# dscripka/openWakeWord

Measured on NVIDIA H100. Metric: 80ms audio-frames/sec (concurrent streams), higher is better.
Workload: dtype f16 operands / f32 accumulate (mel, BN, LayerNorm, sigmoid in f32; heads' first layer as fp16 hi/lo split = f32-grade)

## Files before the change

openwakeword_b200/csrc/cnn_tc.cu:

```cuda
#include "oww_internal.h"
#include "tc_common.cuh"
#include <algorithm>
#include <cmath>
#include <cstring>

namespace {

struct Tc0Args {
    WindowSrc src;
    int n_windows; int T_out;
    const float* w; const float* scale; const float* bias;
    __half* out; int64_t plane;
};

__global__ void __launch_bounds__(256) tc_conv0_kernel(Tc0Args a) {
    __shared__ float s_w[9 * 24];
    __shared__ float s_s[24], s_b[24];
    for (int i = threadIdx.x; i < 9 * 24; i += 256) s_w[i] = a.w[i];
    if (threadIdx.x < 24) { s_s[threadIdx.x] = a.scale[threadIdx.x]; s_b[threadIdx.x] = a.bias[threadIdx.x]; }
    __syncthreads();
    constexpr int Wp = 33;
    const int T = a.T_out;
    const int64_t total = (int64_t)a.n_windows * T * Wp;
    for (int64_t p = (int64_t)blockIdx.x * 256 + threadIdx.x; p < total; p += (int64_t)gridDim.x * 256) {
// ... 230 lines not shown
                        reinterpret_cast<uint32_t*>(o + (int64_t)(a.cg_out + g) * a.out_plane)[q] = lw;
                        if (po == 0) reinterpret_cast<uint32_t*>(o + (int64_t)(a.cg_out + g) * a.out_plane - 1)[q] = 0u;
                    }
                }
            }
        }
    }
}

struct TcBlkArgs {
    const __half* in; LateLay lay;
    const __half* w; const float* scale; const float* bias;
    int n, W, rows_new;
    int m_valid, tap;
    int pool_f;
    int cg_in, cg_out, apply_act, n_tiles;
    float* out_f32;
    __half* out[3]; int out_toff[3];
    LateLay out_lay;
    int64_t out_plane;
};

template <int CGP, int NP>
__global__ void __launch_bounds__(kTcThreads, 1) tc_conv_blk_kernel(TcBlkArgs a) {
    extern __shared__ __align__(128) uint8_t smem[];
    constexpr int W_TERM = 3 * CGP * NP * 16;
    constexpr int W_BYTES = 2 * W_TERM;
    uint8_t* w_smem = smem;
    const int units = a.lay.units;
    const int half_bytes = CGP * units * 16;
    uint8_t* a_smem = smem + W_BYTES;
    uint64_t* bars = reinterpret_cast<uint64_t*>(a_smem + 2 * half_bytes);
    float* s_sb = reinterpret_cast<float*>(bars + 6);
    for (int i = threadIdx.x; i < NP; i += kTcThreads) { s_sb[i] = a.scale[i]; s_sb[NP + i] = a.bias[i]; }

    const int warp = threadIdx.x >> 5, lane = threadIdx.x & 31;
    const uint32_t bar0 = smem_u32(bars);
    auto full_bar = [&](int h) { return bar0 + 8u * h; };
    auto empty_bar = [&](int h) { return bar0 + 8u * (2 + h); };
    const uint32_t wfull_bar = bar0 + 8u * 4;

    if (threadIdx.x == 0) {
        for (int h = 0; h < 2; ++h) { mbar_init(full_bar(h), 1); mbar_init(empty_bar(h), 8); }
        mbar_init(wfull_bar, 1);
        asm volatile("fence.mbarrier_init.release.cluster;" ::: "memory");
    }
    if (a.cg_in < CGP)
        for (int h = 0; h < 2; ++h) {
// ... 54 lines not shown
                        for (int wt = 0; wt < (h == 0 ? 2 : 1); ++wt) {
                            const uint32_t w_t = w_addr + (wt == 1 ? (uint32_t)W_TERM : 0u);
                            const uint64_t ad = make_desc(a_addr + (uint32_t)h * (uint32_t)half_bytes + (uint32_t)(2 * qq) * lbo_a + (uint32_t)j * tap16,
                                                          lbo_a, 128u);
                            const uint64_t bd = make_desc(w_t + (uint32_t)((j * CGP + 2 * qq) * NP) * 16u, NP * 16u, 128u);
                            wg_mma<NP>(acc, ad, bd, (h | j | qq | wt) != 0);
                        }
                    }
                }
                wg_commit();
                wg_wait_all();
                __syncwarp();
                if (lane == 0) mbar_arrive(empty_bar(h));
            }
            phase ^= 1;

#pragma unroll
            for (int i = 0; i < 2; ++i) {
                const int t = tr[i], sl = slr[i], f = fr[i];
                const int n = tile * a.lay.S + sl;
                const bool live = okr[i] && n < a.n;
                if (a.out_f32) {
                    if (!live || f != 0) continue;
                    float* o = a.out_f32 + ((int64_t)n * a.rows_new + t) * 96;
#pragma unroll
                    for (int j = 0; j < NP / 8; ++j) {
                        const int c = j * 8 + 2 * q;
                        if (c >= 96) continue;
                        float2 r;
                        r.x = fmaf(acc[4 * j + 2 * i], s_sb[c], s_sb[NP + c]);
// ... 123 lines not shown
                        8 * (2 * stages + 2) + 2 * NP * sizeof(float);
    if (smem > 227 * 1024) return oww_fail(ctx, OWW_EUNSUPPORTED, "tensor-core conv tile does not fit shared memory (%zu bytes)", smem);
    const uint32_t bit = 1u << (((CGP / 2 + NP / 16) + (TERMS == 3 ? 16 : 0)) & 31);
    if (!(ctx->tc_attr_mask & bit)) {
        OWW_CUDA(ctx, cudaFuncSetAttribute(tc_conv_kernel<CGP, NP, TERMS>, cudaFuncAttributeMaxDynamicSharedMemorySize, 227 * 1024));
        ctx->tc_attr_mask |= bit;
    }
    int grid = ctx->sm_count < a.n_tiles ? ctx->sm_count : a.n_tiles;
    tc_conv_kernel<CGP, NP, TERMS><<<grid, kTcThreads, smem, s>>>(a);
    OWW_LAUNCH_CHECK(ctx);
    return OWW_OK;
}

template <int CGP, int NP>
int launch_tc_blk(oww_ctx* ctx, const TcBlkArgs& a, cudaStream_t s) {
    const size_t smem = (size_t)2 * 3 * CGP * NP * 16 + (size_t)2 * CGP * a.lay.units * 16 + 8 * 6 + 2 * NP * sizeof(float);
    if (smem > 227 * 1024) return oww_fail(ctx, OWW_EUNSUPPORTED, "blocked late conv tile does not fit shared memory (%zu bytes)", smem);
    const uint32_t bit = 1u << (CGP / 2 + NP / 16);
    if (!(ctx->tc_blk_attr_mask & bit)) {
        OWW_CUDA(ctx, cudaFuncSetAttribute(tc_conv_blk_kernel<CGP, NP>, cudaFuncAttributeMaxDynamicSharedMemorySize, 227 * 1024));
        ctx->tc_blk_attr_mask |= bit;
    }
    const int grid = ctx->sm_count < a.n_tiles ? ctx->sm_count : a.n_tiles;
    OWW_CUDA(ctx, oww_launch_pdl(ctx->late_pdl, tc_conv_blk_kernel<CGP, NP>, dim3(grid), dim3(kTcThreads), smem, s, a));
    OWW_LAUNCH_CHECK(ctx);
    return OWW_OK;
}

}

int oww_tc_pack_weights(oww_ctx* ctx, const float* h_blob) {
// ... 161 lines not shown
            if (rc) return rc;
            if (cap->late && (rc = oww_late_capture(ctx, li + 1, bufs[cur ^ 1], in_plane, T, W, s))) return rc;
        }
        if (li == stop_layer && !last) {
            const int64_t total = (int64_t)n * T * W * L.cout;
            tc_unpack_kernel<<<(unsigned)((total + 255) / 256), 256, 0, s>>>(bufs[cur ^ 1], in_plane, d_dbg, n, T, W, L.cout, out_split ? 1 : 0);
            OWW_LAUNCH_CHECK(ctx);
            return OWW_OK;
        }
    }
    return OWW_OK;
}

namespace {

__global__ void late_capture_kernel(const uint4* planes, int64_t plane_pitch, int T, int Wp, int n_planes, uint4* tmpl) {
    const int total = n_planes * 2 * Wp;
    for (int i = blockIdx.x * blockDim.x + threadIdx.x; i < total; i += gridDim.x * blockDim.x) {
        const int f = i % Wp, r = (i / Wp) % 2, pl = i / (2 * Wp);
        tmpl[i] = planes[(int64_t)pl * plane_pitch + kGuard + (int64_t)(T - 2 + r) * Wp + f];
    }
}

}

int oww_late_alloc(oww_ctx* ctx) {
    for (auto& X : ctx->late_x) for (auto& b : X.buf) { cudaFree(b); b = nullptr; }
    cudaFree(ctx->d_late_tmp); ctx->d_late_tmp = nullptr;
    cudaFree(ctx->d_late_template); ctx->d_late_template = nullptr;
    ctx->late_active = false;
// ... 14 lines not shown
        LateLay& Y = X.lay;
        Y.kh3 = kh3 ? 1 : 0; Y.T = rows + (kh3 ? 2 : 0); Y.Wq = kh3 ? W : W + 1;
        Y.S = std::max(1, 128 / (rows * Y.Wq));
        if (kh3) while (Y.S > 1 && Y.T * Y.S * W > 256) Y.S /= 2;
        const int tap = kh3 ? Y.S * W : 1;
        Y.units = round8(std::max((kh3 ? 0 : 1) + Y.T * Y.S * Y.Wq, 2 * tap + 128));
        Y.blk_stride = (int64_t)2 * X.cg * Y.units;
        const size_t buf_units = (size_t)((n + Y.S - 1) / Y.S) * Y.blk_stride;
        X.tmpl_off = kh3 ? (int)tmpl_units : -1;
        if (kh3) tmpl_units += (size_t)2 * X.cg * 2 * (W + 1);
        for (int k = 0; k < X.n_buf; ++k) {
            OWW_CUDA(ctx, cudaMalloc(&X.buf[k], buf_units * 16));
            OWW_CUDA(ctx, cudaMemset(X.buf[k], 0, buf_units * 16));
        }
        if (C.pool_t) {
            const size_t u = (size_t)2 * (C.cout / 8) * ((kGuard + (size_t)n * rows * (W + 1) + kGuardBack + 7) & ~(size_t)7);
            if (u > tmp_units) tmp_units = u;
            rows /= C.pool_t; W /= C.pool_f;
        }
    }
    if (tmp_units) {
        OWW_CUDA(ctx, cudaMalloc(&ctx->d_late_tmp, tmp_units * 16));
        OWW_CUDA(ctx, cudaMemset(ctx->d_late_tmp, 0, tmp_units * 16));
    }
    OWW_CUDA(ctx, cudaMalloc(&ctx->d_late_template, std::max<size_t>(tmpl_units, 1) * 16));
    OWW_CUDA(ctx, cudaMemset(ctx->d_late_template, 0, std::max<size_t>(tmpl_units, 1) * 16));
    ctx->late_step = 0;
    ctx->late_active = true;
    return OWW_OK;
}

int oww_late_chain(oww_ctx* ctx, float* d_emb, cudaStream_t s) {
// ... 12 lines not shown
                toff[m] = 2 - m * Y.rows_new;
            }
        };
        const int64_t tmp_plane = (int64_t)((kGuard + (int64_t)n * T_out * (W + 1) + kGuardBack + 7) & ~7LL);
        TcBlkArgs b;
        std::memset(&b, 0, sizeof(b));
        b.in = reinterpret_cast<const __half*>(X.buf[X.n_buf == 1 ? 0 : (int)(k % X.n_buf)]);
        b.lay = X.lay;
        b.w = reinterpret_cast<const __half*>(ctx->d_tc_w3) + 2 * ctx->tc_w_off[l];
        b.scale = ctx->d_tc_sb3 + ctx->tc_sb_off[l]; b.bias = b.scale + np;
        b.n = n; b.W = W; b.rows_new = T_out;
        b.m_valid = T_out * X.lay.S * X.lay.Wq;
        b.tap = C.kh == 3 ? X.lay.S * W : 1;
        b.cg_in = cg; b.cg_out = C.cout / 8; b.apply_act = last ? 0 : 1;
        b.n_tiles = (n + X.lay.S - 1) / X.lay.S;
        const bool fuse_pool = !last && C.pool_t == 1 && C.pool_f == 2 && X.lay.kh3 && (W & 1) == 0;
        if (last) {
            b.out_f32 = d_emb;
        } else if (C.pool_t && !fuse_pool) {
            b.out[0] = reinterpret_cast<__half*>(ctx->d_late_tmp);
            b.out_plane = tmp_plane;
        } else {
            const oww_ctx::LateTensor& Y = ctx->late_x[l + 1];
            route(Y, b.out, b.out_toff);
            b.out_lay = Y.lay;
            b.pool_f = fuse_pool ? 2 : 0;
        }
        int rc;
        if (cgp == 4 && np == 48) rc = launch_tc_blk<4, 48>(ctx, b, s);
        else if (cgp == 6 && np == 48) rc = launch_tc_blk<6, 48>(ctx, b, s);
        else if (cgp == 6 && np == 80) rc = launch_tc_blk<6, 80>(ctx, b, s);
        else if (cgp == 10 && np == 80) rc = launch_tc_blk<10, 80>(ctx, b, s);
        else if (cgp == 10 && np == 96) rc = launch_tc_blk<10, 96>(ctx, b, s);
        else if (cgp == 12 && np == 96) rc = launch_tc_blk<12, 96>(ctx, b, s);
        else rc = oww_fail(ctx, OWW_EUNSUPPORTED, "no block-major late conv instance for cgp=%d np=%d", cgp, np);
        if (rc) return rc;
        if (C.pool_t && !last && !fuse_pool) {
            const oww_ctx::LateTensor& Y = ctx->late_x[l + 1];
            PoolOut po{{nullptr, nullptr, nullptr}, {0, 0, 0}, Y.lay};
            route(Y, po.p, po.toff);
            const int cgo = C.cout / 8;
// ... 24 lines not shown
```

openwakeword_b200/csrc/cnn_tc_inc.cu:

```cuda
#include "oww_internal.h"
#include "tc_common.cuh"
#include "mel_device.cuh"
#include <cmath>
#include <cstring>
#include <type_traits>

namespace {

constexpr int kIncEpiWarps = 16;
constexpr int kIncThreads = kIncEpiWarps * 32;
constexpr int kIncMaxG = 7;
constexpr int kMelNF = 2;

__device__ __forceinline__ __half2 u32_as_half2(uint32_t v) {
    return __halves2half2(__ushort_as_half((unsigned short)(v & 0xFFFFu)), __ushort_as_half((unsigned short)(v >> 16)));
}

struct IncArgs {
    IncPlan plan;
    const float* mel; const int* mel_count; int64_t mel_stride; int mel_mask; int back;
    const float* w0; const float* s0; const float* b0;
    const uint8_t* wblob;
    const uint4* tails_in; uint4* tails_out;
    float* emb;
// ... 10 lines not shown
    int hring_off, hslot_bytes, hns;
    const Gate* gates; int n_gates;
    uint4* gx; LateLay gx_lay;
};

__device__ __forceinline__ int head_rows(int slot_bytes, int K, int D) {
    const int r = (slot_bytes / (D * 4)) & ~3;
    return r < K ? r : K;
}

template <int kNL>
__global__ void __launch_bounds__(kIncThreads, 1) tc_inc_kernel(const __grid_constant__ IncArgs a) {
    extern __shared__ __align__(128) uint8_t smem[];
    const IncPlan& P = a.plan;
    const int NL = kNL ? kNL : P.n_layers;
    const int G = P.G;
    uint64_t* bars = reinterpret_cast<uint64_t*>(smem);
    float* s_l0 = reinterpret_cast<float*>(smem + 704);
    uint4* act0 = reinterpret_cast<uint4*>(smem + 2048);

    const int warp = __shfl_sync(0xffffffffu, (int)(threadIdx.x >> 5), 0);
    const int lane = threadIdx.x & 31;
    const uint32_t bar0 = smem_u32(bars);
    auto wfull = [&](int i) { return bar0 + 8u * i; };
    const uint32_t tails_bar = bar0 + 8u * 2;
    auto hfull = [&](int i) { return bar0 + 8u * (3 + i); };
    auto hempty = [&](int i) { return bar0 + 8u * (7 + i); };

    if (threadIdx.x == 0) {
        for (int i = 0; i < 2; ++i) mbar_init(wfull(i), 1);
        mbar_init(tails_bar, 1);
        for (int i = 0; i < 4; ++i) { mbar_init(hfull(i), 1); mbar_init(hempty(i), kIncEpiWarps); }
        asm volatile("fence.mbarrier_init.release.cluster;" ::: "memory");
    }
    for (int i = threadIdx.x; i < 9 * 24; i += kIncThreads) s_l0[i] = a.w0[i];
    if (threadIdx.x < 24) { s_l0[216 + threadIdx.x] = a.s0[threadIdx.x]; s_l0[240 + threadIdx.x] = a.b0[threadIdx.x]; }
    asm volatile("fence.proxy.async.shared::cta;" ::: "memory");
    __syncthreads();

    auto load_weights = [&](int l) {
        mbar_expect_tx(wfull(l & 1), (uint32_t)P.L[l].w_bytes);
        bulk_g2s(smem_u32(smem + P.L[l].w_smem), a.wblob + P.L[l].w_off, (uint32_t)P.L[l].w_bytes, wfull(l & 1));
    };
    if (threadIdx.x == 0 && (int)blockIdx.x < P.n_groups) { load_weights(1); load_weights(2); }

    int hq_head = 0, hq_layer = 0, hq_row = 0, hchunk_p = 0;
    auto issue_head_chunk = [&]() -> bool {
        if (hq_head >= a.n_heads) return false;
        const HeadDev& H = a.heads[hq_head];
        const int slot = hchunk_p % a.hns;
        mbar_wait(hempty(slot), ((hchunk_p / a.hns) & 1) ^ 1);
        uint32_t bytes; const float* src;
        if (hq_layer == 0) {
            bytes = (uint32_t)(96 * H.dims[1]) * 4u;
            src = H.blob + H.w_off[0] + (int64_t)hq_row * 96 * H.dims[1];
            if (++hq_row == H.n_in) { hq_row = 0; hq_layer = 1; }
        } else {
            const int K = H.dims[hq_layer], D = H.dims[hq_layer + 1];
            const int rows = head_rows(a.hslot_bytes, K, D);
// ... 13 lines not shown
    uint32_t epi_tails_par = 0, mma_tails_par = 0;
    uint32_t hf_par = 0; int hchunk_e = 0;
    for (int grp = blockIdx.x; grp < P.n_groups; grp += gridDim.x) {
        const uint4* tin = a.tails_in + (int64_t)grp * P.tail_units;
        uint4* tout = a.tails_out + (int64_t)grp * P.tail_units;
        int* s_cnt = reinterpret_cast<int*>(smem + 512);
        int* s_live = s_cnt + 16;
        float* s_mel = reinterpret_cast<float*>(smem + P.scratch_off + 6144);
        if (a.dbg_clock && blockIdx.x == 0 && grp == 0 && et == 0) a.dbg_clock[101] = clock64();
        named_bar_sync(2, kIncEpiWarps * 32);
        if (et < G) {
            const int b = grp * G + et;
            s_live[et] = b < a.B && (!a.live_chunks || a.live_chunks[b] >= a.live_min);
        }
        named_bar_sync(2, kIncEpiWarps * 32);
        if (a.fused) {
            uint8_t* sc = smem + P.scratch_off;
            float2* s_tw = reinterpret_cast<float2*>(sc);
            float* s_win = reinterpret_cast<float*>(sc + 4096);
            uint8_t* s_work = smem + 2048 + warp * (kMelNF * kMelFrameScratch);
            float* s_floor = s_mel + G * 256;
            int seen_v = 1;
            for (int i = et; i < 512; i += kIncEpiWarps * 32) { s_tw[i] = a.mel_twiddle[i]; s_win[i] = a.mel_window[i]; }
            if (et < G) {
                const int b = grp * G + et;
                s_cnt[et] = s_live[et] ? a.mel_count_rw[b] : 0;
                s_cnt[8 + et] = s_live[et] ? a.feat_count[b] : 0;
                seen_v = s_live[et] ? a.seen[b] : 1;
                s_live[8 + et] = s_live[et] && seen_v == 0;
            }
            named_bar_sync(2, kIncEpiWarps * 32);
// ... 90 lines not shown
            if (l == 0) {
                const int Wp = 33, NP2 = 17;
                for (int q = et; q < 8 * G * NP2; q += kIncEpiWarps * 32) {
                    const int j = q % NP2, tg = q / NP2, g = tg % G, t = tg / G;
                    const int f0 = 2 * j;
                    const int b = grp * G + g;
                    uint4* o = nx + 1 + tg * Wp + f0;
                    const uint4 z = make_uint4(0, 0, 0, 0);
                    if (j == 16) { o[0] = z; o[L.nx_pitch] = z; o[2 * L.nx_pitch] = z; continue; }
                    if (!s_live[g]) {
                        o[0] = z; o[L.nx_pitch] = z; o[2 * L.nx_pitch] = z;
                        o[1] = z; o[L.nx_pitch + 1] = z; o[2 * L.nx_pitch + 1] = z;
                        continue;
                    }
                    const float* base = a.mel + (int64_t)b * a.mel_stride;
                    const int row0 = (a.fused ? s_cnt[g] - 2 : a.mel_count[b] - a.back - 10) + t;
                    float x[3][4];
#pragma unroll
                    for (int dt = 0; dt < 3; ++dt) {
                        const float* rp = (a.fused && t + dt >= 2) ? s_mel + (g * 8 + t + dt - 2) * 32
                                                                   : base + (int64_t)((row0 + dt) & a.mel_mask) * 32;
#pragma unroll
                        for (int i = 0; i < 4; ++i) {
                            const int ff = f0 + i - 1;
                            x[dt][i] = (ff >= 0 && ff < 32) ? rp[ff] : 0.f;
                        }
                    }
#pragma unroll
                    for (int pl = 0; pl < 3; ++pl) {
                        __half2 h0[4], h1[4];
#pragma unroll
                        for (int u = 0; u < 4; ++u) {
                            float v0[2], v1[2];
#pragma unroll
                            for (int e = 0; e < 2; ++e) {
// ... 84 lines not shown
                };
                auto epi_item = [&](auto nc_const, auto final_const, const float* acc, int it) {
                    constexpr int NP = decltype(nc_const)::value;
                    constexpr bool kFinal = decltype(final_const)::value;
                    const int t64 = it / n_chunks, c0 = (it - t64 * n_chunks) * NP;
#pragma unroll
                    for (int i = 0; i < 2; ++i) {
                        const int m = t64 * 64 + wq * 16 + (lane >> 2) + 8 * i;
                        if (m >= lM) continue;
                        const int tg = (int)__umulhi((uint32_t)m, wp_magic);
                        const int f = m - tg * lWp;
                        const int g = G > 1 ? tg - (int)__umulhi((uint32_t)tg, g_magic) * G : 0;
                        const bool live = s_live[g] != 0;
                        if constexpr (kFinal) {
                            if (f != 0 || !live) continue;
                            float* o = a.fused ? a.feat_ring + (int64_t)(grp * G + g) * a.feat_stride + (int64_t)(s_cnt[8 + g] & a.feat_mask) * 96
                                               : a.emb + (int64_t)(grp * G + g) * 96;
#pragma unroll
                            for (int j = 0; j < NP / 8; ++j) {
                                const int c = c0 + j * 8 + 2 * q;
                                float2 r;
                                r.x = fmaf(acc[4 * j + 2 * i], sb[c], sb[lnp + c]);
                                r.y = fmaf(acc[4 * j + 2 * i + 1], sb[c + 1], sb[lnp + c + 1]);
                                *reinterpret_cast<float2*>(o + c) = r;
                            }
                            continue;
                        }
                        const bool pad = f == lW;
                        uint4* d0 = dst + (1 + t_off_units + m);
                        const bool keep_tail = !lpool && ltail >= 0 && m >= tail_start && live;
                        uint4* t0 = tout + (ltail + (m - tail_start));
// ... 118 lines not shown
                    }
                }
            }
            if (L.nx_tail_off >= 0) epi_tails_par ^= 1;
            asm volatile("fence.proxy.async.shared::cta;" ::: "memory");
            named_bar_sync(1, kIncEpiWarps * 32);
            if (l > 0 && et == 0) {
                if (l + 2 < NL) load_weights(l + 2);
                else if (grp + (int)gridDim.x < P.n_groups) {
                    if (l == NL - 2 && (l & 1)) load_weights(1);
                    if (l == NL - 1) { if (l & 1) load_weights(1); load_weights(2); }
                }
            }
        }
        if (a.dbg_clock && blockIdx.x == 0 && grp == 0 && et == 0) a.dbg_clock[OWW_N_CONV] = clock64();
        if (a.fused && NL == OWW_N_CONV) {
            named_bar_sync(2, kIncEpiWarps * 32);
            if (a.n_heads > 0) {
            if (et == 0) {
                hq_head = hq_layer = hq_row = 0;
                for (int i = 0; i < a.hns && issue_head_chunk(); ++i) {}
            }
            auto refill_head_ring = [&]() {
                while (hchunk_p < hchunk_e - 1 + max(a.hns, 2) && issue_head_chunk()) {}
            };
            const int NI = a.max_n_in;
            float* feats = reinterpret_cast<float*>(smem + 2048);
            float* red = feats + G * NI * 96;
            float* hA = red + 4 * G * 128;
            float* hB = hA + G * 256;
            for (int i0 = et; i0 < G * NI * 24; i0 += 4 * kIncEpiWarps * 32) {
// ... 279 lines not shown
        if (L.nx_base + size_nx[l] > hi) hi = L.nx_base + size_nx[l];
        act_high[l] = kActBase + hi * 16;
    }
    auto wsz = [&](int l) { return l >= 1 && l < NL ? (P.L[l].w_bytes + 127) & ~127 : 0; };
    for (int l = 1; l < NL; ++l) {
        const int above = wsz(l + 1) > wsz(l - 1) ? wsz(l + 1) : wsz(l - 1);
        P.L[l].w_smem = (l & 1) ? kTop - wsz(l) : kTop - above - wsz(l);
    }
    for (int l = 1; l < NL; ++l) {
        int w_low = P.L[l].w_smem;
        if (l + 1 < NL && P.L[l + 1].w_smem < w_low) w_low = P.L[l + 1].w_smem;
        if (act_high[l] > w_low || act_high[l - 1] > P.L[l].w_smem)
            return oww_fail(ctx, OWW_EUNSUPPORTED, "fused-CNN smem plan does not fit at layer %d (G=%d)", l, G);
        if (l >= 2 && wsz(l) < wsz(l - 1)) return oww_fail(ctx, OWW_EUNSUPPORTED, "weight sizes must not shrink with depth");
    }
    {
        int off = kActBase + r8(size_nx[0]) * 16;
        const int work_end = kActBase + kIncEpiWarps * kMelNF * kMelFrameScratch;
        if (work_end > off) off = (work_end + 127) & ~127;
        const int need_b = 6144 + G * 256 * 4 + 64;
        P.scratch_off = (off + need_b <= P.L[1].w_smem && off + need_b <= P.L[2].w_smem) ? off : 0;
    }
    P.w_total_bytes = (int)w_off;
    P.smem_bytes = kTop;
    *out = P;
    return OWW_OK;
}

int oww_inc_setup(oww_ctx* ctx, const float* h_blob) {
    IncPlan P;
    int rc = oww_inc_build_plan(ctx, 1, 1, OWW_N_CONV, &P);
// ... 76 lines not shown
        for (int l = 0; l <= h.desc.n_layers; ++l) d.dims[l] = h.desc.dims[l];
        for (int l = 0; l < h.desc.n_layers; ++l) {
            d.w_off[l] = (int)h.w_off[l]; d.b_off[l] = (int)h.b_off[l];
            d.g_off[l] = (int)h.g_off[l]; d.h_off[l] = (int)h.h_off[l];
        }
        d.col0 = h.col0;
    }
    cudaFree(ctx->d_head_devs); ctx->d_head_devs = nullptr;
    if (v.empty()) return OWW_OK;
    OWW_CUDA(ctx, cudaMalloc(&ctx->d_head_devs, v.size() * sizeof(HeadDev)));
    OWW_CUDA(ctx, cudaMemcpy(ctx->d_head_devs, v.data(), v.size() * sizeof(HeadDev), cudaMemcpyHostToDevice));
    return OWW_OK;
}

bool oww_fused_frontend_supported(const oww_ctx* ctx) {
    return ctx->fuse_step && ctx->cfg.cnn_mode == OWW_CNN_TC_INCREMENTAL && ctx->inc_plan.scratch_off != 0;
}

bool oww_fused_heads_supported(const oww_ctx* ctx) {
    if (!oww_fused_frontend_supported(ctx) || ctx->heads.empty() || ctx->heads.size() > 16) return false;
    if (ctx->inc_plan.n_layers < OWW_N_CONV) return false;
    {
        size_t w1 = 0;
        for (const Head& h : ctx->heads) w1 += (size_t)h.desc.dims[0] * h.desc.dims[1] * sizeof(float);
        if ((size_t)ctx->inc_plan.n_groups * w1 > ((size_t)256 << 20)) return false;
    }
    for (const Head& h : ctx->heads) {
        if (h.desc.dims[1] > 128) return false;
        for (int l = 1; l <= h.desc.n_layers; ++l) if (h.desc.dims[l] > 256) return false;
    }
    const size_t floats = (size_t)ctx->inc_plan.G * ((size_t)ctx->max_n_in * 96 + 4 * 128 + 2 * 256);
    int d1max = 32;
    for (const Head& h : ctx->heads) d1max = h.desc.dims[1] > d1max ? h.desc.dims[1] : d1max;
    return 2048 + floats * 4 + 128 + (size_t)96 * d1max * 4 <= (size_t)ctx->inc_plan.L[2].w_smem;
}

static void launch_inc(const IncArgs& a, int grid, cudaStream_t s) {
    if (a.plan.n_layers == OWW_N_CONV) tc_inc_kernel<OWW_N_CONV><<<grid, kIncThreads, a.plan.smem_bytes, s>>>(a);
    else if (a.plan.n_layers == 11) tc_inc_kernel<11><<<grid, kIncThreads, a.plan.smem_bytes, s>>>(a);
    else if (a.plan.n_layers == 15) tc_inc_kernel<15><<<grid, kIncThreads, a.plan.smem_bytes, s>>>(a);
    else tc_inc_kernel<0><<<grid, kIncThreads, a.plan.smem_bytes, s>>>(a);
}

static void fill_inc_args(oww_ctx* ctx, IncArgs& a) {
    std::memset(&a, 0, sizeof(a));
    a.plan = ctx->inc_plan;
    a.mel = ctx->d_mel_ring; a.mel_count = ctx->d_mel_count; a.mel_stride = (int64_t)ctx->mel_rows * 32;
    a.mel_mask = ctx->mel_rows - 1;
    a.w0 = ctx->conv[0].d_w; a.s0 = ctx->conv[0].d_scale; a.b0 = ctx->conv[0].d_bias;
    a.wblob = reinterpret_cast<const uint8_t*>(ctx->d_inc_w);
    a.tails_in = reinterpret_cast<const uint4*>(ctx->d_inc_tails[ctx->inc_cur]);
    a.tails_out = reinterpret_cast<uint4*>(ctx->d_inc_tails[ctx->inc_cur ^ 1]);
    a.B = ctx->n_streams;
    a.dbg_clock = reinterpret_cast<long long*>(ctx->d_inc_dbg);
    if (ctx->late_active) {
        a.gx = reinterpret_cast<uint4*>(ctx->late_x[ctx->split_from].buf[0]);
        a.gx_lay = ctx->late_x[ctx->split_from].lay;
    }
}

int oww_fused_step(oww_ctx* ctx, const int16_t* d_pcm, int64_t pcm_stride, float* d_scores, int out_stride, bool with_heads,
                   cudaStream_t s, const int* d_chunks, int min_chunks) {
    IncArgs a;
    fill_inc_args(ctx, a);
    a.live_chunks = d_chunks; a.live_min = min_chunks;
    a.fused = 1;
    a.pcm = d_pcm; a.pcm_stride = pcm_stride;
    a.tail = ctx->d_tail; a.seen = ctx->d_seen; a.mel_rw = ctx->d_mel_ring; a.mel_count_rw = ctx->d_mel_count;
    a.mel_window = ctx->d_window; a.mel_twiddle = ctx->d_twiddle; a.mel_start = ctx->d_mel_start; a.mel_len = ctx->d_mel_len;
    a.mel_w = ctx->d_mel_w; a.mel_kmax = ctx->mel_kmax;
    a.feat_ring = ctx->d_feat_ring; a.feat_stride = (int64_t)ctx->feat_rows * 96; a.feat_mask = ctx->feat_rows - 1;
    a.feat_count = ctx->d_feat_count;
    a.heads = ctx->d_head_devs; a.n_heads = with_heads ? (int)ctx->heads.size() : 0; a.max_n_in = ctx->max_n_in > 0 ? ctx->max_n_in : 1;
    a.scores = d_scores; a.score_stride = out_stride;
    a.gates = ctx->d_gates; a.n_gates = with_heads ? (int)ctx->gates.size() : 0;
    if (with_heads) {
        int d1max = 32;
        for (const Head& h : ctx->heads) d1max = h.desc.dims[1] > d1max ? h.desc.dims[1] : d1max;
        const int G = a.plan.G;
        const int used = 2048 + (G * (a.max_n_in * 96 + 4 * 128 + 2 * 256)) * 4;
        a.hring_off = (used + 127) & ~127;
        a.hslot_bytes = 96 * d1max * 4;
        const int avail = a.plan.L[2].w_smem - a.hring_off;
        a.hns = avail / a.hslot_bytes;
        if (a.hns > 4) a.hns = 4;
        if (a.hns < 1 && !ctx->heads.empty()) return oww_fail(ctx, OWW_EUNSUPPORTED, "no room for the fused heads weight ring");
    }
    const int grid = a.plan.n_groups < ctx->sm_count ? a.plan.n_groups : ctx->sm_count;
    launch_inc(a, grid, s);
    OWW_LAUNCH_CHECK(ctx);
    ctx->inc_cur ^= 1;
    return OWW_OK;
}

int oww_cnn_inc_step(oww_ctx* ctx, int back, float* d_emb, cudaStream_t s, const int* d_chunks, int min_chunks) {
    IncArgs a;
    fill_inc_args(ctx, a);
    a.live_chunks = d_chunks; a.live_min = min_chunks;
    a.back = back;
    a.emb = d_emb;
    const int grid = a.plan.n_groups < ctx->sm_count ? a.plan.n_groups : ctx->sm_count;
    launch_inc(a, grid, s);
    OWW_LAUNCH_CHECK(ctx);
    ctx->inc_cur ^= 1;
    if (ctx->late_active) return oww_late_chain(ctx, d_emb, s);
    return OWW_OK;
}

int oww_inc_capture(oww_ctx* ctx, int layer, const void* planes, int64_t plane_pitch, int T, int W, int win0, int n_win,
                    int stream0, const int* d_ids, cudaStream_t s) {
    const IncLayer& L = ctx->inc_plan.L[layer];
    if (layer >= ctx->inc_plan.n_layers - (ctx->inc_plan.n_layers < OWW_N_CONV ? 1 : 0) || L.nx_tail_off < 0) return OWW_OK;
    const int Wp = W + 1;
    const int64_t total = (int64_t)n_win * L.cg_out * 2 * Wp;
    unsigned grid = (unsigned)((total + 255) / 256);
    tc_capture_kernel<<<grid, 256, 0, s>>>(reinterpret_cast<const uint4*>(planes), plane_pitch, T, Wp, L.cg_out, win0, n_win,
                                          stream0, d_ids, ctx->inc_plan.G, L.nx_tail_off, ctx->inc_plan.tail_units,
// ... 47 lines not shown
```

openwakeword_b200/csrc/mel.cu:

```cuda
#include "oww_internal.h"
#include "mel_device.cuh"
#include <climits>
#include <cmath>
#include <cstring>

namespace {

constexpr int kWarps = 8;
constexpr int kThreads = kWarps * 32;

struct MelDev {
    const float* window;
    const float2* twiddle;
    const int* mel_start;
    const int* mel_len;
    const float* mel_w;
    int kmax;
};

__global__ void __launch_bounds__(kThreads) mel_kernel(MelLaunch p, MelDev c) {
    __shared__ float2 s_buf[kWarps][2][256];
    __shared__ float2 s_tw[512];
    __shared__ float s_win[512];
    __shared__ float s_pow[kWarps][264];
    __shared__ float s_red[kWarps];

    const int clip = p.ids ? p.ids[blockIdx.x] : blockIdx.x;
    const int tid = threadIdx.x, lane = tid & 31, warp = tid >> 5;

    for (int i = tid; i < 512; i += kThreads) { s_tw[i] = c.twiddle[i]; s_win[i] = c.window[i]; }

    const bool streaming = p.tail != nullptr;
    const int prefix = streaming ? OWW_TAIL : 0;
    const bool fresh = streaming && p.seen[clip] == 0;
    const int total = prefix + p.n_body;
    const int T = (total - OWW_FFT_N) / OWW_HOP + 1;
    const int f0 = fresh ? 3 : 0;
    const int16_t* body = p.body + (int64_t)clip * p.body_stride;
    const int16_t* tail = streaming ? p.tail + (int64_t)clip * OWW_TAIL : nullptr;
    const int row0 = p.out_count ? p.out_count[clip] : 0;
    float* out = p.out + (int64_t)clip * p.out_stride;
    __syncthreads();

    const int my_start = c.mel_start[lane];
    const int my_len = c.mel_len[lane];
    const float* my_w = c.mel_w + lane * OWW_MEL_MAXSUPPORT;
    float vmax = -INFINITY;

    for (int f = f0 + warp; f < T; f += kWarps) {
        const float db = mel_frame_db(tail, prefix, body, f, s_buf[warp][0], s_buf[warp][1], s_pow[warp], s_tw, s_win, c.kmax,
                                      my_start, my_len, my_w, lane);
        vmax = fmaxf(vmax, db);
        const int r = f - f0;
        const int slot = p.out_rows_mask >= 0 ? ((row0 + r) & p.out_rows_mask) : r;
        out[(int64_t)slot * OWW_MEL_BINS + lane] = db;
        __syncwarp();
    }
#pragma unroll
    for (int o = 16; o > 0; o >>= 1) vmax = fmaxf(vmax, __shfl_xor_sync(0xffffffffu, vmax, o));
    if (lane == 0) s_red[warp] = vmax;
    __syncthreads();
    float m = s_red[0];
#pragma unroll
    for (int w = 1; w < kWarps; ++w) m = fmaxf(m, s_red[w]);
    const float floor_db = m - 80.0f;
    const int nrows = T - f0;
    for (int i = tid; i < nrows * OWW_MEL_BINS; i += kThreads) {
        const int r = i >> 5, col = i & 31;
        const int slot = p.out_rows_mask >= 0 ? ((row0 + r) & p.out_rows_mask) : r;
        float* q = out + (int64_t)slot * OWW_MEL_BINS + col;
        float v = fmaxf(__ldcg(q), floor_db);
        if (p.affine) v = v / 10.0f + 2.0f;
        *q = v;
    }
    if (streaming) {
        __syncthreads();
        int16_t* tw = p.tail + (int64_t)clip * OWW_TAIL;
        for (int i = tid; i < OWW_TAIL; i += kThreads) tw[i] = __ldg(body + (p.n_body - OWW_TAIL + i));
        if (tid == 0) {
            p.out_count[clip] = oww_wrap_count(row0 + nrows);
            const int sn = p.seen[clip] + p.n_chunks;
            p.seen[clip] = sn > (1 << 30) ? (1 << 30) : sn;
        }
    }
}

__host__ __device__ __forceinline__ int clip_frame_step(int f) { return f < 5 ? 0 : (f - 5) / 8 + 1; }
__host__ __device__ __forceinline__ int clip_group(int f, int chunk) {
    return (int)oww_call_first_step(oww_call_of_step(clip_frame_step(f), chunk), chunk);
}
__host__ __device__ __forceinline__ int clip_first_group(int k0, int chunk) { return clip_group(8 * k0 > 71 ? 8 * k0 - 71 : 0, chunk); }

__global__ void __launch_bounds__(kThreads) mel_clip_kernel(const int16_t* pcm, const int64_t* clip_off, const int* clip_len, int pad,
                                                            int chunk, int k0, int k1, float* out, int64_t out_stride, MelDev c) {
    extern __shared__ __align__(16) uint8_t dyn[];
    float2 (*s_buf)[2][256] = reinterpret_cast<float2 (*)[2][256]>(dyn);
// ... 52 lines not shown
}
double mel_to_hz(double m) {
    const double f_sp = 200.0 / 3.0, min_log_hz = 1000.0, min_log_mel = min_log_hz / f_sp;
    const double logstep = std::log(6.4) / 27.0;
    return m >= min_log_mel ? min_log_hz * std::exp(logstep * (m - min_log_mel)) : f_sp * m;
}

}

int oww_mel_launch(oww_ctx* ctx, const MelLaunch& p, cudaStream_t s) {
    if (!ctx->mel_loaded) return oww_fail(ctx, OWW_EINVAL, "mel constants not loaded");
    const int prefix = p.tail ? OWW_TAIL : 0;
    if (prefix + p.n_body < OWW_FFT_N) return oww_fail(ctx, OWW_EINVAL, "clip shorter than 512 samples");
    if (p.n_clips <= 0) return OWW_OK;
    MelDev c{ctx->d_window, ctx->d_twiddle, ctx->d_mel_start, ctx->d_mel_len, ctx->d_mel_w, ctx->mel_kmax};
    mel_kernel<<<p.n_clips, kThreads, 0, s>>>(p, c);
    OWW_LAUNCH_CHECK(ctx);
    return OWW_OK;
}

int oww_mel_clips_launch(oww_ctx* ctx, const int16_t* d_pcm, const int64_t* d_off, const int* d_len, int n_clips, int pad,
                         int chunk, int k0, int k1, float* d_out, int64_t out_stride, cudaStream_t s) {
    if (!ctx->mel_loaded) return oww_fail(ctx, OWW_EINVAL, "mel constants not loaded");
    if (n_clips <= 0 || k1 <= k0) return OWW_OK;
    if (k0 < 0 || k1 - k0 > 8192 || chunk < 1 || oww_call_first_step(oww_call_of_step(k1, chunk), chunk) != k1)
        return oww_fail(ctx, OWW_EINVAL, "step range [%d,%d) is not a bulk frontend segment", k0, k1);
    MelDev c{ctx->d_window, ctx->d_twiddle, ctx->d_mel_start, ctx->d_mel_len, ctx->d_mel_w, ctx->mel_kmax};
    const size_t smem = (size_t)kWarps * 2 * 256 * sizeof(float2) + 512 * sizeof(float2) + 512 * sizeof(float) +
                        (size_t)kWarps * 264 * sizeof(float) + (size_t)kWarps * 512 * sizeof(int16_t) +
                        (size_t)(k1 - clip_first_group(k0, chunk)) * sizeof(int);
    if (!ctx->mel_clip_attr_set) {
// ... 73 lines not shown
```

openwakeword_b200/csrc/mel_device.cuh:

```cuda
#pragma once
#include <cuda_runtime.h>
#include <cstdint>
#include "oww_internal.h"

namespace {

__device__ __forceinline__ float2 cmul(float2 a, float2 b) {
    return make_float2(__fmaf_rn(a.x, b.x, -__fmul_rn(a.y, b.y)), __fmaf_rn(a.x, b.y, __fmul_rn(a.y, b.x)));
}

template <bool kBodyGlobal = true>
__device__ __forceinline__ float mel_frame_db(const int16_t* tail, int prefix, const int16_t* body, int f, float2* a, float2* b,
                                              float* pw_buf, const float2* s_tw, const float* s_win, int kmax, int my_start,
                                              int my_len, const float* my_w, int lane) {
#pragma unroll
        for (int j = 0; j < 8; ++j) {
            const int n = lane + 32 * j;
            const int s0 = f * OWW_HOP + 2 * n;
            float x0, x1;
            if (s0 + 1 < prefix) { x0 = (float)tail[s0]; x1 = (float)tail[s0 + 1]; }
            else if (s0 >= prefix) {
                if (kBodyGlobal) { x0 = (float)__ldg(body + (s0 - prefix)); x1 = (float)__ldg(body + (s0 + 1 - prefix)); }
                else { x0 = (float)body[s0 - prefix]; x1 = (float)body[s0 + 1 - prefix]; }
            }
// ... 49 lines not shown
        const float db = 10.0f * logf(fmaxf(acc, 1e-10f)) / logf(10.0f);
    return db;
}

#ifndef OWW_FFT_SWZ
#define OWW_FFT_SWZ 1
#endif
__device__ __forceinline__ int fswz(int e) {
#if OWW_FFT_SWZ
    return e ^ (((e >> 4) & 3) * 5);
#else
    return e;
#endif
}

constexpr int kMelFrameScratch = 2048 + 2048 + 1280;
template <int NF>
__device__ __forceinline__ void mel_frames_db(const int16_t* const* tail, int prefix, const int16_t* const* body, const int* f,
                                              uint8_t* bufs, const float2* s_tw, const float* s_win, int kmax, int my_start,
                                              int my_len, const float* my_w, int lane, float* db, long long* stamps = nullptr) {
    float2* a[NF]; float2* b[NF]; float* pw[NF];
    if (stamps && lane == 0) stamps[0] = clock64();
#pragma unroll
    for (int i = 0; i < NF; ++i) {
        a[i] = reinterpret_cast<float2*>(bufs + i * kMelFrameScratch);
        b[i] = a[i] + 256;
        pw[i] = reinterpret_cast<float*>(b[i] + 256);
    }
    bool al[NF];
#pragma unroll
    for (int i = 0; i < NF; ++i) al[i] = (((size_t)body[i] | (size_t)tail[i]) & 3) == 0 && (prefix & 1) == 0;
    uint32_t raw[8][NF];
#pragma unroll
    for (int j = 0; j < 8; ++j) {
        const int n = lane + 32 * j;
#pragma unroll
        for (int i = 0; i < NF; ++i) {
            const int s0 = f[i] * OWW_HOP + 2 * n;
            if (al[i]) {
                raw[j][i] = s0 + 1 < prefix ? *reinterpret_cast<const uint32_t*>(tail[i] + s0)
                                            : __ldg(reinterpret_cast<const uint32_t*>(body[i] + (s0 - prefix)));
            } else {
// ... 97 lines not shown
```

openwakeword_b200/csrc/oww_internal.h:

```cpp
#pragma once
#include <cuda_runtime.h>
#include <algorithm>
#include <cmath>
#include <cstdint>
#include <cstdio>
#include <string>
#include <utility>
#include <vector>
#include "owwb200.h"

__host__ __device__ inline int oww_scale_exponent_of_max(float amax, int lo = -8, int hi = 24) {
    if (!(amax > 0.f) || !(amax <= 3.402823466e38f)) return 0;
    int e;
    frexpf(amax, &e);
    e = 14 - e;
    return e < lo ? lo : (e > hi ? hi : e);
}
inline int oww_weight_scale_exponent(const float* w, size_t n) {
    float amax = 0.f;
    for (size_t i = 0; i < n; ++i) amax = std::fmax(amax, std::fabs(w[i]));
    return oww_scale_exponent_of_max(amax);
}

#define OWW_N_CONV 20
// ... 293 lines not shown
#else
#define OWW_HD inline
#endif
OWW_HD int64_t oww_clip_calls(int64_t L, int c) { return L > c ? (L - 1) / c : 0; }
OWW_HD int64_t oww_call_first_step(int64_t j, int c) { return j * c / OWW_SAMPLES_PER_CHUNK; }
OWW_HD int64_t oww_call_of_step(int64_t s, int c) { return ((int64_t)OWW_SAMPLES_PER_CHUNK * (s + 1) + c - 1) / c - 1; }

struct MelLaunch {
    const int16_t* body; int64_t body_stride; int n_body;
    int16_t* tail;
    int* seen;
    float* out; int64_t out_stride; int out_rows_mask;
    int* out_count;
    int n_clips; int affine; int n_chunks;
    const int* ids = nullptr;
};
int oww_mel_launch(oww_ctx* ctx, const MelLaunch& p, cudaStream_t s);
int oww_mel_clips_launch(oww_ctx* ctx, const int16_t* d_pcm, const int64_t* d_off, const int* d_len, int n_clips, int pad,
                         int chunk, int k0, int k1, float* d_out, int64_t out_stride, cudaStream_t s);

struct WindowSrc {
    const float* base; int64_t stride;
    const int* count; int rows_mask;
    int n_streams; int n_chunks;
    const int* ids = nullptr;
};
int oww_feat_append(oww_ctx* ctx, const float* d_emb, int n_chunks, cudaStream_t s, const int* d_ids = nullptr, int n_ids = 0);
int oww_cnn_window(oww_ctx* ctx, const WindowSrc& src, int n_windows, float* d_emb, cudaStream_t s, bool capture_tails = false);
int oww_cnn_fp32_pyramid(oww_ctx* ctx, const WindowSrc& src, int n, int T0, float* d_emb, int out_rows, int stop_layer,
                         float* d_dbg, cudaStream_t s);
// ... 99 lines not shown
```

Measured before the change: 5.676 million.

## Fuse 2x2 max-pool into late conv epilogue, add PDL to mel and incremental kernels

Adds a fused time-and-frequency max-pool path to the blocked late conv epilogue. It pools across lanes with shuffles and across warpgroups through shared memory, so the pooled layer no longer writes and rereads a temporary buffer. Separately, the mel kernel moves to the shared mel_frames_db scratch layout with a smaller buffer, gains a one-pass register path, skips inactive streams, and supports programmatic dependent launch. The incremental CNN kernel also gets a non-fused path that runs mel first and then launches the CNN with PDL overlap. The extra barriers and shared memory in the conv epilogue, plus PDL ordering, add risks around correctness and occupancy.

```diff
diff --git a/openwakeword_b200/csrc/cnn_tc.cu b/openwakeword_b200/csrc/cnn_tc.cu
--- a/openwakeword_b200/csrc/cnn_tc.cu
+++ b/openwakeword_b200/csrc/cnn_tc.cu
@@ -268,6 +268,7 @@
     int n, W, rows_new;
     int m_valid, tap;
     int pool_f;
+    int pool_t;
     int cg_in, cg_out, apply_act, n_tiles;
     float* out_f32;
     __half* out[3]; int out_toff[3];
@@ -286,6 +287,7 @@
     uint8_t* a_smem = smem + W_BYTES;
     uint64_t* bars = reinterpret_cast<uint64_t*>(a_smem + 2 * half_bytes);
     float* s_sb = reinterpret_cast<float*>(bars + 6);
+    float* s_x = s_sb + 2 * NP;
     for (int i = threadIdx.x; i < NP; i += kTcThreads) { s_sb[i] = a.scale[i]; s_sb[NP + i] = a.bias[i]; }
 
     const int warp = threadIdx.x >> 5, lane = threadIdx.x & 31;
@@ -370,6 +372,58 @@
                 if (lane == 0) mbar_arrive(empty_bar(h));
             }
             phase ^= 1;
+
+            if (a.pool_t == 2) {
+                const bool fw = ((lane >> 2) & 1) == 0;
+                const int ci = wq * 16 + (lane >> 3) * 4 + (lane & 3);
+#pragma unroll
+                for (int i = 0; i < 2; ++i)
+#pragma unroll
+                    for (int j = 0; j < NP / 8; ++j) {
+                        const int c = j * 8 + 2 * q;
+                        float y0 = fmaf(acc[4 * j + 2 * i], s_sb[c], s_sb[NP + c]);
+                        float y1 = fmaf(acc[4 * j + 2 * i + 1], s_sb[c + 1], s_sb[NP + c + 1]);
+                        if (a.apply_act) { y0 = act(y0); y1 = act(y1); }
+                        acc[4 * j + 2 * i] = fmaxf(y0, __shfl_xor_sync(0xffffffffu, y0, 4));
+                        acc[4 * j + 2 * i + 1] = fmaxf(y1, __shfl_xor_sync(0xffffffffu, y1, 4));
+                    }
+                if (wg == 1 && fw) {
+#pragma unroll
+                    for (int k = 0; k < NP / 2; ++k) s_x[k * 64 + ci] = acc[k];
+                }
+                named_bar_sync(1, 256);
+                if (wg == 0 && fw) {
+#pragma unroll
+                    for (int i = 0; i < 2; ++i) {
+                        const int sl = slr[i], fo = fr[i] >> 1;
+                        const int n = tile * a.lay.S + sl;
+                        if (!okr[i] || n >= a.n) continue;
+                        uint4* dst[3];
+#pragma unroll
+                        for (int kk = 0; kk < 3; ++kk)
+                            dst[kk] = a.out[kk] && a.out_toff[kk] >= 0
+                                          ? reinterpret_cast<uint4*>(a.out[kk]) + late_unit(a.out_lay, 0, n, a.out_toff[kk], fo) : nullptr;
+#pragma unroll
+                        for (int j = 0; j < NP / 8; ++j) {
+                            if (j >= a.cg_out) break;
+                            const float y0 = fmaxf(acc[4 * j + 2 * i], s_x[(4 * j + 2 * i) * 64 + ci]);
+                            const float y1 = fmaxf(acc[4 * j + 2 * i + 1], s_x[(4 * j + 2 * i + 1) * 64 + ci]);
+                            const __half h0 = __float2half_rn(y0), h1 = __float2half_rn(y1);
+                            const __half2 hh = __halves2half2(h0, h1);
+                            const __half2 ll = __floats2half2_rn(y0 - __half2float(h0), y1 - __half2float(h1));
+                            const uint32_t hw = *reinterpret_cast<const uint32_t*>(&hh), lw = *reinterpret_cast<const uint32_t*>(&ll);
+#pragma unroll
+                            for (int kk = 0; kk < 3; ++kk)
+                                if (dst[kk]) {
+                                    reinterpret_cast<uint32_t*>(dst[kk] + (int64_t)j * a.out_lay.units)[q] = hw;
+                                    reinterpret_cast<uint32_t*>(dst[kk] + (int64_t)(a.cg_out + j) * a.out_lay.units)[q] = lw;
+                                }
+                        }
+                    }
+                }
+                named_bar_sync(2, 256);
+                continue;
+            }
 
 #pragma unroll
             for (int i = 0; i < 2; ++i) {
@@ -523,7 +577,8 @@
 
 template <int CGP, int NP>
 int launch_tc_blk(oww_ctx* ctx, const TcBlkArgs& a, cudaStream_t s) {
-    const size_t smem = (size_t)2 * 3 * CGP * NP * 16 + (size_t)2 * CGP * a.lay.units * 16 + 8 * 6 + 2 * NP * sizeof(float);
+    const size_t smem = (size_t)2 * 3 * CGP * NP * 16 + (size_t)2 * CGP * a.lay.units * 16 + 8 * 6 + 2 * NP * sizeof(float) +
+                        (a.pool_t == 2 ? (size_t)NP / 2 * 64 * sizeof(float) : 0);
     if (smem > 227 * 1024) return oww_fail(ctx, OWW_EUNSUPPORTED, "blocked late conv tile does not fit shared memory (%zu bytes)", smem);
     const uint32_t bit = 1u << (CGP / 2 + NP / 16);
     if (!(ctx->tc_blk_attr_mask & bit)) {
@@ -715,6 +770,12 @@
 
 namespace {
 
+int late_fused_pool_t(const ConvLayer& C, const LateLay& X, int rows, int W, bool last) {
+    if (last || !C.pool_t || C.pool_f != 2 || !X.kh3 || (W & 1)) return 0;
+    if (C.pool_t == 1) return 1;
+    return C.pool_t == 2 && rows == 2 && X.S * W == 64 ? 2 : 0;
+}
+
 __global__ void late_capture_kernel(const uint4* planes, int64_t plane_pitch, int T, int Wp, int n_planes, uint4* tmpl) {
     const int total = n_planes * 2 * Wp;
     for (int i = blockIdx.x * blockDim.x + threadIdx.x; i < total; i += gridDim.x * blockDim.x) {
@@ -759,8 +820,10 @@
             OWW_CUDA(ctx, cudaMemset(X.buf[k], 0, buf_units * 16));
         }
         if (C.pool_t) {
-            const size_t u = (size_t)2 * (C.cout / 8) * ((kGuard + (size_t)n * rows * (W + 1) + kGuardBack + 7) & ~(size_t)7);
-            if (u > tmp_units) tmp_units = u;
+            if (!late_fused_pool_t(C, Y, rows, W, l == OWW_N_CONV - 1)) {
+                const size_t u = (size_t)2 * (C.cout / 8) * ((kGuard + (size_t)n * rows * (W + 1) + kGuardBack + 7) & ~(size_t)7);
+                if (u > tmp_units) tmp_units = u;
+            }
             rows /= C.pool_t; W /= C.pool_f;
         }
     }
@@ -803,7 +866,8 @@
         b.tap = C.kh == 3 ? X.lay.S * W : 1;
         b.cg_in = cg; b.cg_out = C.cout / 8; b.apply_act = last ? 0 : 1;
         b.n_tiles = (n + X.lay.S - 1) / X.lay.S;
-        const bool fuse_pool = !last && C.pool_t == 1 && C.pool_f == 2 && X.lay.kh3 && (W & 1) == 0;
+        const int fused_pool_t = late_fused_pool_t(C, X.lay, T_out, W, last);
+        const bool fuse_pool = fused_pool_t != 0;
         if (last) {
             b.out_f32 = d_emb;
         } else if (C.pool_t && !fuse_pool) {
@@ -814,6 +878,7 @@
             route(Y, b.out, b.out_toff);
             b.out_lay = Y.lay;
             b.pool_f = fuse_pool ? 2 : 0;
+            b.pool_t = fused_pool_t == 2 ? 2 : 0;
         }
         int rc;
         if (cgp == 4 && np == 48) rc = launch_tc_blk<4, 48>(ctx, b, s);
diff --git a/openwakeword_b200/csrc/cnn_tc_inc.cu b/openwakeword_b200/csrc/cnn_tc_inc.cu
--- a/openwakeword_b200/csrc/cnn_tc_inc.cu
+++ b/openwakeword_b200/csrc/cnn_tc_inc.cu
@@ -48,6 +48,7 @@
     extern __shared__ __align__(128) uint8_t smem[];
     const IncPlan& P = a.plan;
     const int NL = kNL ? kNL : P.n_layers;
+    const bool fused = kNL == OWW_N_CONV && a.fused;
     const int G = P.G;
     uint64_t* bars = reinterpret_cast<uint64_t*>(smem);
     float* s_l0 = reinterpret_cast<float*>(smem + 704);
@@ -77,6 +78,7 @@
         bulk_g2s(smem_u32(smem + P.L[l].w_smem), a.wblob + P.L[l].w_off, (uint32_t)P.L[l].w_bytes, wfull(l & 1));
     };
     if (threadIdx.x == 0 && (int)blockIdx.x < P.n_groups) { load_weights(1); load_weights(2); }
+    pdl_wait();
 
     int hq_head = 0, hq_layer = 0, hq_row = 0, hchunk_p = 0;
     auto issue_head_chunk = [&]() -> bool {
@@ -120,7 +122,7 @@
             s_live[et] = b < a.B && (!a.live_chunks || a.live_chunks[b] >= a.live_min);
         }
         named_bar_sync(2, kIncEpiWarps * 32);
-        if (a.fused) {
+        if (fused) {
             uint8_t* sc = smem + P.scratch_off;
             float2* s_tw = reinterpret_cast<float2*>(sc);
             float* s_win = reinterpret_cast<float*>(sc + 4096);
@@ -241,11 +243,11 @@
                         continue;
                     }
                     const float* base = a.mel + (int64_t)b * a.mel_stride;
-                    const int row0 = (a.fused ? s_cnt[g] - 2 : a.mel_count[b] - a.back - 10) + t;
+                    const int row0 = (fused ? s_cnt[g] - 2 : a.mel_count[b] - a.back - 10) + t;
                     float x[3][4];
 #pragma unroll
                     for (int dt = 0; dt < 3; ++dt) {
-                        const float* rp = (a.fused && t + dt >= 2) ? s_mel + (g * 8 + t + dt - 2) * 32
+                        const float* rp = (fused && t + dt >= 2) ? s_mel + (g * 8 + t + dt - 2) * 32
                                                                    : base + (int64_t)((row0 + dt) & a.mel_mask) * 32;
 #pragma unroll
                         for (int i = 0; i < 4; ++i) {
@@ -360,7 +362,7 @@
                         const bool live = s_live[g] != 0;
                         if constexpr (kFinal) {
                             if (f != 0 || !live) continue;
-                            float* o = a.fused ? a.feat_ring + (int64_t)(grp * G + g) * a.feat_stride + (int64_t)(s_cnt[8 + g] & a.feat_mask) * 96
+                            float* o = fused ? a.feat_ring + (int64_t)(grp * G + g) * a.feat_stride + (int64_t)(s_cnt[8 + g] & a.feat_mask) * 96
                                                : a.emb + (int64_t)(grp * G + g) * 96;
 #pragma unroll
                             for (int j = 0; j < NP / 8; ++j) {
@@ -509,7 +511,7 @@
             }
         }
         if (a.dbg_clock && blockIdx.x == 0 && grp == 0 && et == 0) a.dbg_clock[OWW_N_CONV] = clock64();
-        if (a.fused && NL == OWW_N_CONV) {
+        if (fused) {
             named_bar_sync(2, kIncEpiWarps * 32);
             if (a.n_heads > 0) {
             if (et == 0) {
@@ -819,7 +821,7 @@
             return oww_fail(ctx, OWW_EUNSUPPORTED, "fused-CNN smem plan does not fit at layer %d (G=%d)", l, G);
         if (l >= 2 && wsz(l) < wsz(l - 1)) return oww_fail(ctx, OWW_EUNSUPPORTED, "weight sizes must not shrink with depth");
     }
-    {
+    if (NL == OWW_N_CONV) {
         int off = kActBase + r8(size_nx[0]) * 16;
         const int work_end = kActBase + kIncEpiWarps * kMelNF * kMelFrameScratch;
         if (work_end > off) off = (work_end + 127) & ~127;
@@ -926,7 +928,8 @@
 }
 
 bool oww_fused_frontend_supported(const oww_ctx* ctx) {
-    return ctx->fuse_step && ctx->cfg.cnn_mode == OWW_CNN_TC_INCREMENTAL && ctx->inc_plan.scratch_off != 0;
+    return ctx->fuse_step && ctx->cfg.cnn_mode == OWW_CNN_TC_INCREMENTAL &&
+           (ctx->inc_plan.n_layers < OWW_N_CONV || ctx->inc_plan.scratch_off != 0);
 }
 
 bool oww_fused_heads_supported(const oww_ctx* ctx) {
@@ -947,11 +950,12 @@
     return 2048 + floats * 4 + 128 + (size_t)96 * d1max * 4 <= (size_t)ctx->inc_plan.L[2].w_smem;
 }
 
-static void launch_inc(const IncArgs& a, int grid, cudaStream_t s) {
-    if (a.plan.n_layers == OWW_N_CONV) tc_inc_kernel<OWW_N_CONV><<<grid, kIncThreads, a.plan.smem_bytes, s>>>(a);
-    else if (a.plan.n_layers == 11) tc_inc_kernel<11><<<grid, kIncThreads, a.plan.smem_bytes, s>>>(a);
-    else if (a.plan.n_layers == 15) tc_inc_kernel<15><<<grid, kIncThreads, a.plan.smem_bytes, s>>>(a);
-    else tc_inc_kernel<0><<<grid, kIncThreads, a.plan.smem_bytes, s>>>(a);
+static cudaError_t launch_inc(const IncArgs& a, int grid, cudaStream_t s, bool pdl = false) {
+    void (*k)(IncArgs) = a.plan.n_layers == OWW_N_CONV ? tc_inc_kernel<OWW_N_CONV>
+                       : a.plan.n_layers == 11         ? tc_inc_kernel<11>
+                       : a.plan.n_layers == 15         ? tc_inc_kernel<15>
+                                                       : tc_inc_kernel<0>;
+    return oww_launch_pdl(pdl, k, dim3(grid), dim3(kIncThreads), (size_t)a.plan.smem_bytes, s, a);
 }
 
 static void fill_inc_args(oww_ctx* ctx, IncArgs& a) {
@@ -976,6 +980,18 @@
     IncArgs a;
     fill_inc_args(ctx, a);
     a.live_chunks = d_chunks; a.live_min = min_chunks;
+    const int grid = a.plan.n_groups < ctx->sm_count ? a.plan.n_groups : ctx->sm_count;
+    if (a.plan.n_layers < OWW_N_CONV) {
+        MelLaunch m{d_pcm, pcm_stride, OWW_SAMPLES_PER_CHUNK, ctx->d_tail, ctx->d_seen, ctx->d_mel_ring,
+                    (int64_t)ctx->mel_rows * 32, ctx->mel_rows - 1, ctx->d_mel_count, ctx->n_streams, 1, 1};
+        m.live = d_chunks; m.live_min = min_chunks; m.pdl = ctx->late_pdl;
+        int rc = oww_mel_launch(ctx, m, s);
+        if (rc) return rc;
+        OWW_CUDA(ctx, launch_inc(a, grid, s, ctx->late_pdl));
+        OWW_LAUNCH_CHECK(ctx);
+        ctx->inc_cur ^= 1;
+        return OWW_OK;
+    }
     a.fused = 1;
     a.pcm = d_pcm; a.pcm_stride = pcm_stride;
     a.tail = ctx->d_tail; a.seen = ctx->d_seen; a.mel_rw = ctx->d_mel_ring; a.mel_count_rw = ctx->d_mel_count;
@@ -998,8 +1014,7 @@
         if (a.hns > 4) a.hns = 4;
         if (a.hns < 1 && !ctx->heads.empty()) return oww_fail(ctx, OWW_EUNSUPPORTED, "no room for the fused heads weight ring");
     }
-    const int grid = a.plan.n_groups < ctx->sm_count ? a.plan.n_groups : ctx->sm_count;
-    launch_inc(a, grid, s);
+    OWW_CUDA(ctx, launch_inc(a, grid, s));
     OWW_LAUNCH_CHECK(ctx);
     ctx->inc_cur ^= 1;
     return OWW_OK;
@@ -1012,7 +1027,7 @@
     a.back = back;
     a.emb = d_emb;
     const int grid = a.plan.n_groups < ctx->sm_count ? a.plan.n_groups : ctx->sm_count;
-    launch_inc(a, grid, s);
+    OWW_CUDA(ctx, launch_inc(a, grid, s));
     OWW_LAUNCH_CHECK(ctx);
     ctx->inc_cur ^= 1;
     if (ctx->late_active) return oww_late_chain(ctx, d_emb, s);
diff --git a/openwakeword_b200/csrc/mel.cu b/openwakeword_b200/csrc/mel.cu
--- a/openwakeword_b200/csrc/mel.cu
+++ b/openwakeword_b200/csrc/mel.cu
@@ -1,4 +1,5 @@
 #include "oww_internal.h"
+#include "tc_common.cuh"
 #include "mel_device.cuh"
 #include <climits>
 #include <cmath>
@@ -18,24 +19,31 @@
     int kmax;
 };
 
-__global__ void __launch_bounds__(kThreads) mel_kernel(MelLaunch p, MelDev c) {
-    __shared__ float2 s_buf[kWarps][2][256];
+__global__ void __launch_bounds__(kThreads, 5) mel_kernel(MelLaunch p, MelDev c) {
+    __shared__ __align__(16) uint8_t s_work[kWarps][kMelFrameScratch];
     __shared__ float2 s_tw[512];
     __shared__ float s_win[512];
-    __shared__ float s_pow[kWarps][264];
     __shared__ float s_red[kWarps];
 
+    pdl_trigger();
     const int clip = p.ids ? p.ids[blockIdx.x] : blockIdx.x;
     const int tid = threadIdx.x, lane = tid & 31, warp = tid >> 5;
+    if (p.live && p.live[clip] < p.live_min) {
+        pdl_wait();
+        return;
+    }
 
     for (int i = tid; i < 512; i += kThreads) { s_tw[i] = c.twiddle[i]; s_win[i] = c.window[i]; }
 
     const bool streaming = p.tail != nullptr;
     const int prefix = streaming ? OWW_TAIL : 0;
-    const bool fresh = streaming && p.seen[clip] == 0;
+    const int seen0 = streaming ? p.seen[clip] : 0;
+    const bool fresh = streaming && seen0 == 0;
     const int total = prefix + p.n_body;
     const int T = (total - OWW_FFT_N) / OWW_HOP + 1;
     const int f0 = fresh ? 3 : 0;
+    const int nrows = T - f0;
+    const bool one_pass = nrows <= kWarps;
     const int16_t* body = p.body + (int64_t)clip * p.body_stride;
     const int16_t* tail = streaming ? p.tail + (int64_t)clip * OWW_TAIL : nullptr;
     const int row0 = p.out_count ? p.out_count[clip] : 0;
@@ -45,16 +53,17 @@
     const int my_start = c.mel_start[lane];
     const int my_len = c.mel_len[lane];
     const float* my_w = c.mel_w + lane * OWW_MEL_MAXSUPPORT;
-    float vmax = -INFINITY;
+    float vmax = -INFINITY, kept = 0.f;
 
     for (int f = f0 + warp; f < T; f += kWarps) {
-        const float db = mel_frame_db(tail, prefix, body, f, s_buf[warp][0], s_buf[warp][1], s_pow[warp], s_tw, s_win, c.kmax,
-                                      my_start, my_len, my_w, lane);
+        float db;
+        mel_frames_db<1>(&tail, prefix, &body, &f, s_work[warp], s_tw, s_win, c.kmax, my_start, my_len, my_w, lane, &db);
         vmax = fmaxf(vmax, db);
+        if (one_pass) { kept = db; continue; }
+        pdl_wait();
         const int r = f - f0;
         const int slot = p.out_rows_mask >= 0 ? ((row0 + r) & p.out_rows_mask) : r;
         out[(int64_t)slot * OWW_MEL_BINS + lane] = db;
-        __syncwarp();
     }
 #pragma unroll
     for (int o = 16; o > 0; o >>= 1) vmax = fmaxf(vmax, __shfl_xor_sync(0xffffffffu, vmax, o));
@@ -64,22 +73,38 @@
 #pragma unroll
     for (int w = 1; w < kWarps; ++w) m = fmaxf(m, s_red[w]);
     const float floor_db = m - 80.0f;
-    const int nrows = T - f0;
-    for (int i = tid; i < nrows * OWW_MEL_BINS; i += kThreads) {
-        const int r = i >> 5, col = i & 31;
-        const int slot = p.out_rows_mask >= 0 ? ((row0 + r) & p.out_rows_mask) : r;
-        float* q = out + (int64_t)slot * OWW_MEL_BINS + col;
-        float v = fmaxf(__ldcg(q), floor_db);
-        if (p.affine) v = v / 10.0f + 2.0f;
-        *q = v;
+    int16_t tv[(OWW_TAIL + kThreads - 1) / kThreads];
+#pragma unroll
+    for (int u = 0; u < (OWW_TAIL + kThreads - 1) / kThreads; ++u) {
+        const int i = tid + u * kThreads;
+        tv[u] = streaming && i < OWW_TAIL ? __ldg(body + (p.n_body - OWW_TAIL + i)) : (int16_t)0;
+    }
+    pdl_wait();
+    if (one_pass) {
+        if (warp < nrows) {
+            float v = fmaxf(kept, floor_db);
+            if (p.affine) v = v / 10.0f + 2.0f;
+            const int slot = p.out_rows_mask >= 0 ? ((row0 + warp) & p.out_rows_mask) : warp;
+            out[(int64_t)slot * OWW_MEL_BINS + lane] = v;
+        }
+    } else {
+        for (int i = tid; i < nrows * OWW_MEL_BINS; i += kThreads) {
+            const int r = i >> 5, col = i & 31;
+            const int slot = p.out_rows_mask >= 0 ? ((row0 + r) & p.out_rows_mask) : r;
+            float* q = out + (int64_t)slot * OWW_MEL_BINS + col;
+            float v = fmaxf(__ldcg(q), floor_db);
+            if (p.affine) v = v / 10.0f + 2.0f;
+            *q = v;
+        }
     }
     if (streaming) {
-        __syncthreads();
         int16_t* tw = p.tail + (int64_t)clip * OWW_TAIL;
-        for (int i = tid; i < OWW_TAIL; i += kThreads) tw[i] = __ldg(body + (p.n_body - OWW_TAIL + i));
+#pragma unroll
+        for (int u = 0; u < (OWW_TAIL + kThreads - 1) / kThreads; ++u)
+            if (tid + u * kThreads < OWW_TAIL) tw[tid + u * kThreads] = tv[u];
         if (tid == 0) {
             p.out_count[clip] = oww_wrap_count(row0 + nrows);
-            const int sn = p.seen[clip] + p.n_chunks;
+            const int sn = seen0 + p.n_chunks;
             p.seen[clip] = sn > (1 << 30) ? (1 << 30) : sn;
         }
     }
@@ -162,7 +187,7 @@
     if (prefix + p.n_body < OWW_FFT_N) return oww_fail(ctx, OWW_EINVAL, "clip shorter than 512 samples");
     if (p.n_clips <= 0) return OWW_OK;
     MelDev c{ctx->d_window, ctx->d_twiddle, ctx->d_mel_start, ctx->d_mel_len, ctx->d_mel_w, ctx->mel_kmax};
-    mel_kernel<<<p.n_clips, kThreads, 0, s>>>(p, c);
+    OWW_CUDA(ctx, oww_launch_pdl(p.pdl, mel_kernel, dim3(p.n_clips), dim3(kThreads), 0, s, p, c));
     OWW_LAUNCH_CHECK(ctx);
     return OWW_OK;
 }
diff --git a/openwakeword_b200/csrc/mel_device.cuh b/openwakeword_b200/csrc/mel_device.cuh
--- a/openwakeword_b200/csrc/mel_device.cuh
+++ b/openwakeword_b200/csrc/mel_device.cuh
@@ -87,7 +87,7 @@
 #endif
 }
 
-constexpr int kMelFrameScratch = 2048 + 2048 + 1280;
+constexpr int kMelFrameScratch = 2048 + 2048;
 template <int NF>
 __device__ __forceinline__ void mel_frames_db(const int16_t* const* tail, int prefix, const int16_t* const* body, const int* f,
                                               uint8_t* bufs, const float2* s_tw, const float* s_win, int kmax, int my_start,
@@ -98,7 +98,7 @@
     for (int i = 0; i < NF; ++i) {
         a[i] = reinterpret_cast<float2*>(bufs + i * kMelFrameScratch);
         b[i] = a[i] + 256;
-        pw[i] = reinterpret_cast<float*>(b[i] + 256);
+        pw[i] = reinterpret_cast<float*>(b[i]);
     }
     bool al[NF];
 #pragma unroll
diff --git a/openwakeword_b200/csrc/oww_internal.h b/openwakeword_b200/csrc/oww_internal.h
--- a/openwakeword_b200/csrc/oww_internal.h
+++ b/openwakeword_b200/csrc/oww_internal.h
@@ -331,6 +331,9 @@
     int* out_count;
     int n_clips; int affine; int n_chunks;
     const int* ids = nullptr;
+    const int* live = nullptr;
+    int live_min = 0;
+    bool pdl = false;
 };
 int oww_mel_launch(oww_ctx* ctx, const MelLaunch& p, cudaStream_t s);
 int oww_mel_clips_launch(oww_ctx* ctx, const int16_t* d_pcm, const int64_t* d_off, const int* d_len, int n_clips, int pad,
```

Measured after the change: 6.167 million (median of 6 runs). +8.7%, better.
